# Tcadart/pyLatticeDSO

Hardware: AMD Instinct MI355X
Metric: beams/s assembly+PCG-solve (higher is better)
Workload: dtype f64

## Files before the change

pylatticedso_amd/csrc/pl_coarse.h:

```cpp
#pragma once
#include <hip/hip_runtime.h>

#include <algorithm>
#include <cstdint>
#include <cstdlib>
#include <vector>

#include "pl_dense.h"
#include "pl_kernels.h"
#include "pl_nodeword.h"
#include "pl_tile.h"

namespace pl {

constexpr int kDclMax = 256;
constexpr int kDclSlots = 4096;
inline bool node_words_enabled() {
  const char *e = std::getenv("PL_NODE_WORDS");
  return !(e && e[0] == '0');
}

struct Coarse {
  bool enabled = false;
  bool ready = false;
// ... 700 lines not shown
          mode_disp(q, rela, uA, tA);
          uA = mask3(uA, fa);
          tA = mask3(tA, fa >> 3);
        }
        if (inb) {
          mode_disp(q, relb, uB, tB);
          uB = mask3(uB, fb);
          tB = mask3(tB, fb >> 3);
        }
        V3 F, M;
        tip_force(r, uA, tA, uB, tB, F, M);
        double x6[6] = {0, 0, 0, 0, 0, 0};
        if (inb) {
          const V3 FB = mask3(F, fb), MB = mask3(M, fb >> 3);
          x6[0] += FB.x;
          x6[1] += FB.y;
          x6[2] += FB.z;
          x6[3] += MB.x + (relb[1] * FB.z - relb[2] * FB.y);
          x6[4] += MB.y + (relb[2] * FB.x - relb[0] * FB.z);
          x6[5] += MB.z + (relb[0] * FB.y - relb[1] * FB.x);
        }
        if (ina) {
          const V3 FA = mask3((-1.0) * F, fa), MA = mask3((-1.0) * M - cross(d, F), fa >> 3);
          x6[0] += FA.x;
          x6[1] += FA.y;
          x6[2] += FA.z;
          x6[3] += MA.x + (rela[1] * FA.z - rela[2] * FA.y);
          x6[4] += MA.y + (rela[2] * FA.x - rela[0] * FA.z);
          x6[5] += MA.z + (rela[0] * FA.y - rela[1] * FA.x);
        }
#pragma unroll
        for (int p = 0; p <= q; ++p) RR[q * (q + 1) / 2 + p] += x6[p];
      }
    }
  }
  const int lane = threadIdx.x & 63, wv = threadIdx.x >> 6;
  double *B = raw + (size_t)t * 144;
  if (RIGID) {
#pragma unroll
    for (int e = 0; e < 21; ++e) {
      const double s0 = wave_sum(RR[e]);
      if (lane == 0) red[e][wv] = s0;
    }
    __syncthreads();
    if (threadIdx.x < 21) {
      double v = 0.0;
#pragma unroll
      for (int q = 0; q < kBlock / kWave; ++q) v += red[threadIdx.x][q];
      int q = 0;
      while ((q + 1) * (q + 2) / 2 <= (int)threadIdx.x) ++q;
      const int p = (int)threadIdx.x - q * (q + 1) / 2;
      B[p * 12 + q] = v;
      B[q * 12 + p] = v;
    }
    return;
  }
#pragma unroll
  for (int e = 0; e < 21; ++e) {
    const double s1 = wave_sum(SS[e]);
    if (lane == 0) red[e][wv] = s1;
  }
#pragma unroll
  for (int e = 0; e < (RIGID ? 1 : 36); ++e) {
    const double s2 = wave_sum(RS[e]);
    if (lane == 0) red[21 + e][wv] = s2;
  }
  __syncthreads();
  if (threadIdx.x < 57) {
    double v = 0.0;
#pragma unroll
    for (int q = 0; q < kBlock / kWave; ++q) v += red[threadIdx.x][q];
    if (threadIdx.x < 21) {
      int q = 0;
      while ((q + 1) * (q + 2) / 2 <= (int)threadIdx.x) ++q;
      const int p = (int)threadIdx.x - q * (q + 1) / 2;
      B[(6 + p) * 12 + 6 + q] = v;
      B[(6 + q) * 12 + 6 + p] = v;
    } else {
      const int e = (int)threadIdx.x - 21, p = e / 6, q = e % 6;
      B[p * 12 + 6 + q] = v;
      B[(6 + q) * 12 + p] = v;
    }
  }
}
constexpr int kInv12Block = 192;
__global__ __launch_bounds__(kInv12Block) void k_tile_invert12(int64_t T, const double *__restrict__ raw,
                                                              double *__restrict__ Bt_inv) {
  constexpr int n = 12;
  __shared__ double A[n][n + 1];
  __shared__ double diag0[n];
  const int64_t t = blockIdx.x;
  if (t >= T) return;
  const int e = threadIdx.x, i = e / n, j = e - n * i;
  const bool act = e < n * n;
  if (act) A[i][j] = 0.5 * (raw[t * 144 + i * n + j] + raw[t * 144 + j * n + i]);
  __syncthreads();
  if (e < n) diag0[e] = A[e][e];
  __syncthreads();
  unsigned dropped = 0u;
  for (int k = 0; k < n; ++k) {
    const double d = A[k][k];
    if (!(d > 1e-10 * diag0[k]) || !(diag0[k] > 0.0)) {
      dropped |= 1u << k;
      continue;
    }
    const double inv = 1.0 / d;
    double v = 0.0;
    if (act) {
      const bool di = (dropped >> i) & 1u, dj = (dropped >> j) & 1u;
      if (i == k && j == k) v = -inv;
      else if (i == k) v = A[k][j] * inv;
      else if (j == k) v = A[k][i] * inv;
      else if (di || dj) v = A[i][j];
      else v = A[i][j] - (A[i][k] * inv) * A[k][j];
    }
    __syncthreads();
    if (act) A[i][j] = v;
    __syncthreads();
  }
  if (act) {
    const bool out = ((dropped >> i) & 1u) || ((dropped >> j) & 1u);
    Bt_inv[t * 144 + i * n + j] = out ? 0.0 : -A[i][j];
  }
}
inline void coarse_factor(Coarse &cs, int n, hipStream_t s, const std::function<void(int)> &after_chol, unsigned *bar,
                          TrtriPhases ph = TrtriPhases()) {
  if (cs.w16)
    dense_factor_inverse(cs.Ac, cs.Lf, reinterpret_cast<bf16_t *>(cs.W), reinterpret_cast<bf16_t *>(cs.Wt), cs.Dinv, n, n,
                         cs.info, cs.bw_blocks, s, after_chol, bar, ph);
  else
    dense_factor_inverse(cs.Ac, cs.Lf, cs.W, cs.Wt, cs.Dinv, n, n, cs.info, cs.bw_blocks, s, after_chol, bar, ph);
}
constexpr int kOneGemvMaxDofs = 2048;
inline void coarse_apply(const Coarse &cs, const double *r, double *t, double *y, double *dot_out, const double *add0,
                         hipStream_t s) {
  static const bool one_off = [] { const char *e = std::getenv("PL_ONE_GEMV"); return e && e[0] == '0'; }();
  if (cs.ainv_ready && cs.Ainv && cs.ncp <= kOneGemvMaxDofs && !one_off) {
    hipLaunchKernelGGL(k_full_gemv, dim3((cs.ncp + 3) / 4), dim3(kBlock), 0, s, cs.ncp, (const float *)cs.Ainv, cs.ncp, r, y,
                       dot_out, add0);
    return;
  }
  if (cs.w16)
    dense_apply(reinterpret_cast<const bf16_t *>(cs.W), reinterpret_cast<const bf16_t *>(cs.Wt), cs.ncp, cs.ncp, r, t, y,
                dot_out, add0, s);
  else
    dense_apply(cs.W, cs.Wt, cs.ncp, cs.ncp, r, t, y, dot_out, add0, s);
}

__global__ __launch_bounds__(kBlock) void k_to_float(int64_t n, const double *__restrict__ x, float *__restrict__ y) {
  const int64_t i = (int64_t)blockIdx.x * kBlock + threadIdx.x;
  if (i < n) y[i] = (float)x[i];
}

__device__ __forceinline__ void nword_rel(uint32_t w, double rscale, double &rx, double &ry, double &rz) {
  rx = (double)((int)(w << 24) >> 24) * rscale;
  ry = (double)((int)(w << 16) >> 24) * rscale;
  rz = (double)((int)(w << 8) >> 24) * rscale;
}

template <typename PT, typename RT, int TM = 6, bool MULTI = true, bool LOCAL = true>
__global__ __launch_bounds__(kBlock) void k_pcg_update_tile(const int32_t *__restrict__ tile_start,
                                                            const int32_t *__restrict__ agg_of_tile,
                                                            const double *__restrict__ cen,
                                                            const double *__restrict__ xyz,
                                                            const PT *__restrict__ Ap,
                                                            const float *__restrict__ dinv32,
                                                            const double *__restrict__ w ,
                                                            RT *__restrict__ r,
                                                            double *__restrict__ scal, double *__restrict__ rc,
                                                            const double *__restrict__ Bt_inv ,
                                                            double *__restrict__ yt,
                                                            const int32_t *__restrict__ aggL_of_tile ,
                                                            const double *__restrict__ cenL,
                                                            const uint8_t *__restrict__ shared ,
                                                            double *__restrict__ rcL, int ncp,
                                                            const uint8_t *__restrict__ skip_rows ,
                                                            int cm = 6 ,
                                                            const float *__restrict__ rel32 = nullptr ,
                                                            const uint32_t *__restrict__ nword = nullptr ,
                                                            const uint32_t *__restrict__ dtab = nullptr ,
                                                            double rscale = 0.0 ) {
  __shared__ double red[32][4 * kBlock / kWave];
  if constexpr (!MULTI) {
    w = nullptr;
    shared = nullptr;
  }
  if constexpr (!MULTI || !LOCAL) aggL_of_tile = nullptr;
  double *rr_slot = rc + ncp + (blockIdx.x & (kSlots - 1)), *rdr_slot = rr_slot + kSlots;
  const int t = blockIdx.x;
  double pap, old_rz;
  scalar_read2(scal, S_PAP, S_RZ_OLD, pap, old_rz);
  const double alpha = (pap != 0.0) ? old_rz / pap : 0.0;
  const int n0 = tile_start[t], n1 = tile_start[t + 1];
  const int a = agg_of_tile[t];
  const double c0 = cen[3 * a], c1 = cen[3 * a + 1], c2 = cen[3 * a + 2];
  __shared__ double sbi[16][TM];
  double bi[TM];
#pragma unroll
  for (int j = 0; j < TM; ++j) bi[j] = 0.0;
  const int my_mode = (TM == 12) ? ((int)threadIdx.x < 6 ? (int)threadIdx.x : ((int)threadIdx.x >= 8 && (int)threadIdx.x < 14
                                                                                   ? (int)threadIdx.x - 2 : -1))
                                 : ((int)threadIdx.x < 6 ? (int)threadIdx.x : -1);
  if (Bt_inv && my_mode >= 0) {
#pragma unroll
    for (int j = 0; j < TM; ++j) bi[j] = Bt_inv[(size_t)t * (TM * TM) + TM * my_mode + j];
  }
  if (threadIdx.x < 16) {
#pragma unroll
    for (int j = 0; j < TM; ++j) sbi[threadIdx.x][j] = bi[j];
  }
  double accS[6] = {0, 0, 0, 0, 0, 0};
  double accD[6] = {0, 0, 0, 0, 0, 0};
  double acc[8] = {0, 0, 0, 0, 0, 0, 0, 0};
  const int aL = aggL_of_tile ? aggL_of_tile[t] : 0;
  double l0 = 0.0, l1 = 0.0, l2 = 0.0;
  if (aggL_of_tile) {
    l0 = cenL[3 * aL];
    l1 = cenL[3 * aL + 1];
    l2 = cenL[3 * aL + 2];
  }
  double accL[6] = {0, 0, 0, 0, 0, 0};
  double accT[6] = {0, 0, 0, 0, 0, 0};
  const bool own_t = Bt_inv && shared;
  for (int i = n0 + threadIdx.x; i < n1; i += blockDim.x) {
    if (skip_rows && skip_rows[i]) continue;
    double av[6], dv[6], rv[6];
    const uint32_t nw = nword ? nword[i] : 0u;
    const float2 *d2 = dtab ? reinterpret_cast<const float2 *>(dtab + 8 * (nw >> 24))
                            : reinterpret_cast<const float2 *>(dinv32 + 6 * (int64_t)i);
#pragma unroll
    for (int k = 0; k < 3; ++k) {
      const double2 aa = load_pair(Ap, 3 * (int64_t)i + k), rr = load_pair(r, 3 * (int64_t)i + k);
      const float2 dd = d2[k];
      av[2 * k] = aa.x; av[2 * k + 1] = aa.y;
      dv[2 * k] = dd.x; dv[2 * k + 1] = dd.y;
      rv[2 * k] = rr.x; rv[2 * k + 1] = rr.y;
    }
#pragma unroll
    for (int k = 0; k < 6; ++k) rv[k] -= alpha * av[k];
#pragma unroll
    for (int k = 0; k < 3; ++k) store_pair(r, 3 * (int64_t)i + k, double2{rv[2 * k], rv[2 * k + 1]});
    if (sizeof(RT) == 4) {
#pragma unroll
      for (int k = 0; k < 6; ++k) rv[k] = (double)(float)rv[k];
    }
    double wt[6] = {1, 1, 1, 1, 1, 1};
    if (w) {
#pragma unroll
      for (int k = 0; k < 6; ++k) wt[k] = w[6 * (int64_t)i + k];
    }
    double rx, ry, rz;
    if (rscale != 0.0) {
      nword_rel(nw, rscale, rx, ry, rz);
    } else if (rel32) {
      rx = (double)rel32[3 * (int64_t)i];
      ry = (double)rel32[3 * (int64_t)i + 1];
      rz = (double)rel32[3 * (int64_t)i + 2];
    } else {
      rx = xyz[3 * (int64_t)i] - c0;
      ry = xyz[3 * (int64_t)i + 1] - c1;
      rz = xyz[3 * (int64_t)i + 2] - c2;
    }
    const double ru[3] = {wt[0] * rv[0], wt[1] * rv[1], wt[2] * rv[2]};
    acc[0] += ru[0];
    acc[1] += ru[1];
    acc[2] += ru[2];
    acc[3] += wt[3] * rv[3] + (ry * ru[2] - rz * ru[1]);
    acc[4] += wt[4] * rv[4] + (rz * ru[0] - rx * ru[2]);
    acc[5] += wt[5] * rv[5] + (rx * ru[1] - ry * ru[0]);
#pragma unroll
    for (int k = 0; k < 6; ++k) {
      acc[6] += wt[k] * rv[k] * rv[k];
      acc[7] += wt[k] * dv[k] * rv[k] * rv[k];
    }
    if (TM == 12 && cm == 12 && shared) {
      accD[0] += rx * ru[0];
      accD[1] += ry * ru[1];
      accD[2] += rz * ru[2];
      accD[3] += 0.5 * (ry * ru[0] + rx * ru[1]);
      accD[4] += 0.5 * (rz * ru[1] + ry * ru[2]);
      accD[5] += 0.5 * (rz * ru[0] + rx * ru[2]);
    }
    if (TM == 12 && !(shared && shared[i])) {
      accS[0] += rx * ru[0];
      accS[1] += ry * ru[1];
      accS[2] += rz * ru[2];
      accS[3] += 0.5 * (ry * ru[0] + rx * ru[1]);
      accS[4] += 0.5 * (rz * ru[1] + ry * ru[2]);
      accS[5] += 0.5 * (rz * ru[0] + rx * ru[2]);
    }
    if (own_t && !shared[i]) {
      accT[0] += rv[0];
      accT[1] += rv[1];
      accT[2] += rv[2];
      accT[3] += rv[3] + (ry * rv[2] - rz * rv[1]);
      accT[4] += rv[4] + (rz * rv[0] - rx * rv[2]);
      accT[5] += rv[5] + (rx * rv[1] - ry * rv[0]);
    }
    if (aggL_of_tile && !(shared && shared[i])) {
      const double sx = xyz[3 * (int64_t)i] - l0, sy = xyz[3 * (int64_t)i + 1] - l1, sz = xyz[3 * (int64_t)i + 2] - l2;
      accL[0] += rv[0];
      accL[1] += rv[1];
      accL[2] += rv[2];
      accL[3] += rv[3] + (sy * rv[2] - sz * rv[1]);
      accL[4] += rv[4] + (sz * rv[0] - sx * rv[2]);
      accL[5] += rv[5] + (sx * rv[1] - sy * rv[0]);
// ... 245 lines not shown
  unsigned long long h = 0x9E3779B97F4A7C15ull;
#pragma unroll
  for (int k = 0; k < 7; ++k) {
    h = (h ^ v[k]) * 0xBF58476D1CE4E5B9ull;
    h ^= h >> 29;
  }
  h *= 0x94D049BB133111EBull;
  h ^= h >> 32;
  return h == ~0ull ? 0 : h;
}
__device__ __forceinline__ int dcl_probe(unsigned long long h, unsigned long long *__restrict__ keys,
                                         int *__restrict__ owner, int i) {
  unsigned slot = (unsigned)(h >> 52) & (unsigned)(kDclSlots - 1);
  for (int probe = 0; probe < 32; ++probe) {
    unsigned long long cur = __hip_atomic_load(keys + slot, __ATOMIC_RELAXED, __HIP_MEMORY_SCOPE_AGENT);
    if (cur == ~0ull) cur = atomicCAS(keys + slot, ~0ull, h);
    if (cur == ~0ull || cur == h) {
      if (i < __hip_atomic_load(owner + slot, __ATOMIC_RELAXED, __HIP_MEMORY_SCOPE_AGENT)) atomicMin(owner + slot, i);
      return (int)slot;
    }
    slot = (slot + 1) & (unsigned)(kDclSlots - 1);
  }
  return -1;
}
__global__ __launch_bounds__(kBlock) void k_dcl_insert(int64_t N, const float *__restrict__ dinv,
                                                       const uint8_t *__restrict__ fixedbits,
                                                       unsigned long long *__restrict__ keys, int *__restrict__ owner,
                                                       uint16_t *__restrict__ slot_of_node, int *__restrict__ flags) {
  const int64_t i = (int64_t)blockIdx.x * kBlock + threadIdx.x;
  const bool valid = i < N;
  uint32_t v[7] = {0, 0, 0, 0, 0, 0, 0};
  if (valid) dcl_row(dinv, fixedbits, i, v);
  const unsigned long long h = valid ? dcl_hash(v) : 0ull;
  const int lane = threadIdx.x & 63;
  int found = -2;
  unsigned long long todo = __ballot(valid);
  for (int round = 0; round < 12 && todo; ++round) {
    const int leader = __ffsll((long long)todo) - 1;
    const unsigned long long hl =
        ((unsigned long long)(unsigned)__builtin_amdgcn_readlane((int)(h >> 32), leader) << 32) |
        (unsigned long long)(unsigned)__builtin_amdgcn_readlane((int)(h & 0xFFFFFFFFull), leader);
    const unsigned long long same = __ballot(valid && found == -2 && h == hl);
    int sl = 0;
    if (lane == leader) sl = dcl_probe(h, keys, owner, (int)i);
    sl = __builtin_amdgcn_readlane(sl, leader);
    if ((same >> lane) & 1ull) found = sl;
    todo &= ~same;
  }
  if (valid && found == -2) found = dcl_probe(h, keys, owner, (int)i);
  if (valid) {
    if (found < 0) flags[0] = 1;
    slot_of_node[i] = (uint16_t)(found < 0 ? 0 : found);
  }
}
__global__ __launch_bounds__(kBlock) void k_dcl_publish(int64_t N, const float *__restrict__ dinv,
                                                        const uint8_t *__restrict__ fixedbits,
                                                        const int *__restrict__ owner,
                                                        const uint16_t *__restrict__ slot_of_node,
                                                        int *__restrict__ dense_of_slot, uint32_t *__restrict__ table,
                                                        int *__restrict__ flags) {
  const int64_t i = (int64_t)blockIdx.x * kBlock + threadIdx.x;
  if (i >= N) return;
  const int slot = slot_of_node[i];
  if (owner[slot] != (int)i) return;
  const int d = atomicAdd(flags + 1, 1);
  if (d >= kDclMax) {
    flags[0] = 1;
    return;
  }
  uint32_t v[7];
  dcl_row(dinv, fixedbits, i, v);
#pragma unroll
  for (int k = 0; k < 7; ++k) table[8 * d + k] = v[k];
  table[8 * d + 7] = 0u;
  dense_of_slot[slot] = d;
}
__global__ __launch_bounds__(kBlock) void k_dcl_verify(int64_t N, const float *__restrict__ dinv,
                                                       const uint8_t *__restrict__ fixedbits,
                                                       const uint16_t *__restrict__ slot_of_node,
                                                       const int *__restrict__ dense_of_slot,
                                                       const uint32_t *__restrict__ table, uint32_t *__restrict__ nword,
                                                       int *__restrict__ flags) {
  const int64_t i = (int64_t)blockIdx.x * kBlock + threadIdx.x;
  if (i >= N) return;
  const int d = dense_of_slot[slot_of_node[i]];
  if (d < 0 || d >= kDclMax) {
    flags[0] = 1;
    return;
  }
  uint32_t v[7];
  dcl_row(dinv, fixedbits, i, v);
  bool same = true;
#pragma unroll
  for (int k = 0; k < 7; ++k) same = same && table[8 * d + k] == v[k];
  if (!same) {
    flags[0] = 1;
    return;
  }
  nword[i] = (nword[i] & 0x00FFFFFFu) | ((uint32_t)d << 24);
}
template <typename VT>
__global__ __launch_bounds__(kBlock) void k_condense_subtract(int64_t N, const uint8_t *__restrict__ cflag,
                                                              const VT *__restrict__ y, VT *__restrict__ r) {
  const int64_t t = (int64_t)blockIdx.x * kBlock + threadIdx.x;
  if (t >= 6 * N) return;
  if (!cflag[t / 6]) r[t] = (VT)((double)r[t] - (double)y[t]);
}
template <typename VT>
__global__ __launch_bounds__(kBlock) void k_condense_backsubst(int64_t nc, const int32_t *__restrict__ cnodes,
                                                               const double *__restrict__ inv,
                                                               const uint16_t *__restrict__ cls,
                                                               const VT *__restrict__ b,
                                                               const VT *__restrict__ y, VT *__restrict__ x) {
  const int64_t t = (int64_t)blockIdx.x * kBlock + threadIdx.x;
  const int64_t q = t / 6;
  const int k = (int)(t - 6 * q);
  if (q >= nc) return;
  const int64_t i = cnodes[q];
  const double *A = inv + 36 * (cls ? (int64_t)cls[q] : q);
  double acc = 0.0;
#pragma unroll
  for (int j = 0; j < 6; ++j) acc += A[6 * k + j] * ((double)b[6 * i + j] - (double)y[6 * i + j]);
  x[6 * i + k] = (VT)acc;
}

template <typename PT, typename RT, int TM = 6, bool MULTI = true, bool LOCAL = true>
__global__ __launch_bounds__(kBlock) void k_pcg_direction_coarse(const int32_t *__restrict__ tile_start,
                                                                 const RT *__restrict__ r,
                                                                 const float *__restrict__ dinv32,
                                                                 const double *__restrict__ xyz,
                                                                 const int32_t *__restrict__ agg_of_tile,
                                                                 const double *__restrict__ cen,
                                                                 const double *__restrict__ yc,
                                                                 const double *__restrict__ yt ,
                                                                 const uint8_t *__restrict__ fixedbits,
                                                                 PT *__restrict__ p, RT *__restrict__ x,
                                                                 const double *__restrict__ scal,
                                                                 double *__restrict__ scal_next,
                                                                 double *__restrict__ hist, int k,
                                                                 double *__restrict__ rc, int ncp,
                                                                 const int32_t *__restrict__ aggL_of_tile ,
                                                                 const double *__restrict__ cenL,
                                                                 const double *__restrict__ ycL,
                                                                 const uint8_t *__restrict__ shared ,
                                                                 double *__restrict__ rcL, int ncpL,
                                                                 const uint8_t *__restrict__ zero_rows ,
                                                                 int cm = 6,
                                                                 const float *__restrict__ rel32 = nullptr ,
                                                                 const uint32_t *__restrict__ nword = nullptr,
                                                                 const uint32_t *__restrict__ dtab = nullptr,
                                                                 double rscale = 0.0 ) {
  if constexpr (!MULTI) shared = nullptr;
  if constexpr (!MULTI || !LOCAL) aggL_of_tile = nullptr;
  double old, rz_new, pap;
  scalar_read3(scal, S_RZ_OLD, S_RZ_NEW, S_PAP, old, rz_new, pap);
  const double beta = (old != 0.0) ? rz_new / old : 0.0;
  const double alpha = (pap != 0.0) ? old / pap : 0.0;
  if (blockIdx.x == 1 || gridDim.x == 1)
    for (int e = threadIdx.x; e < ncp; e += blockDim.x) rc[e] = 0.0;
  if (aggL_of_tile && (blockIdx.x == 2 || gridDim.x <= 2))
    for (int e = threadIdx.x; e < ncpL; e += blockDim.x) rcL[e] = 0.0;
  if (blockIdx.x == 0 && threadIdx.x < kWave) {
    const int s = threadIdx.x;
    double rr = 0.0;
    for (int q = s; q < kSlots; q += kWave) rr += rc[ncp + q];
    rr = wave_sum(rr);
    if (s == 0) hist[k] = rr;
    for (int q = s; q < kSlots; q += kWave) {
      rc[ncp + q] = 0.0;
      rc[ncp + kSlots + q] = 0.0;
      scal_next[S_RZ_OLD * kSlots + q] = scal[S_RZ_NEW * kSlots + q];
      scal_next[S_RZ_NEW * kSlots + q] = 0.0;
      scal_next[S_PAP * kSlots + q] = 0.0;
    }
  }
  const int t = blockIdx.x;
  const int n0 = tile_start[t], n1 = tile_start[t + 1];
  const int a = agg_of_tile[t];
  const double *y = yc + cm * a;
  double U0 = y[0], U1 = y[1], U2 = y[2], W0 = y[3], W1 = y[4], W2 = y[5];
  double T[TM];
#pragma unroll
  for (int k = 0; k < TM; ++k) T[k] = 0.0;
  if (yt) {
    const double *q = yt + TM * (size_t)t;
#pragma unroll
    for (int k = 0; k < TM; ++k) T[k] = q[k];
    if (!shared) {
      U0 += T[0]; U1 += T[1]; U2 += T[2]; W0 += T[3]; W1 += T[4]; W2 += T[5];
    }
  }
  double ED[6] = {0, 0, 0, 0, 0, 0};
  if constexpr (TM == 12) {
    if (cm == 12) {
#pragma unroll
      for (int k = 0; k < 6; ++k) ED[k] = y[6 + k];
      if (!shared) {
#pragma unroll
        for (int k = 0; k < 6; ++k) {
          T[6 + k] += ED[k];
          ED[k] = 0.0;
        }
      }
    }
  }
  const bool own_t = yt && shared;
  const double c0 = cen[3 * a], c1 = cen[3 * a + 1], c2 = cen[3 * a + 2];
  double L[6] = {0, 0, 0, 0, 0, 0}, l0 = 0.0, l1 = 0.0, l2 = 0.0;
  if (aggL_of_tile) {
    const int aL = aggL_of_tile[t];
#pragma unroll
    for (int q = 0; q < 6; ++q) L[q] = ycL[6 * aL + q];
    l0 = cenL[3 * aL];
    l1 = cenL[3 * aL + 1];
    l2 = cenL[3 * aL + 2];
  }
  for (int64_t i = n0 + threadIdx.x; i < n1; i += blockDim.x) {
    if (zero_rows && zero_rows[i]) continue;
    const uint32_t nw = nword ? nword[i] : 0u;
    double rx, ry, rz;
    if (rscale != 0.0) {
      nword_rel(nw, rscale, rx, ry, rz);
    } else if (rel32) {
      rx = (double)rel32[3 * i];
      ry = (double)rel32[3 * i + 1];
      rz = (double)rel32[3 * i + 2];
    } else {
      rx = xyz[3 * i] - c0;
      ry = xyz[3 * i + 1] - c1;
      rz = xyz[3 * i + 2] - c2;
    }
    double zc[6] = {U0 + (W1 * rz - W2 * ry), U1 + (W2 * rx - W0 * rz), U2 + (W0 * ry - W1 * rx), W0, W1, W2};
    if constexpr (TM == 12) {
     if (shared && cm == 12) {
      zc[0] += ED[0] * rx + 0.5 * (ED[3] * ry + ED[5] * rz);
      zc[1] += ED[1] * ry + 0.5 * (ED[3] * rx + ED[4] * rz);
      zc[2] += ED[2] * rz + 0.5 * (ED[4] * ry + ED[5] * rx);
     }
     if (!(shared && shared[i])) {
      zc[0] += T[6] * rx + 0.5 * (T[9] * ry + T[11] * rz);
      zc[1] += T[7] * ry + 0.5 * (T[9] * rx + T[10] * rz);
      zc[2] += T[8] * rz + 0.5 * (T[10] * ry + T[11] * rx);
     }
    }
    if (own_t && !shared[i]) {
      zc[0] += T[0] + (T[4] * rz - T[5] * ry);
      zc[1] += T[1] + (T[5] * rx - T[3] * rz);
      zc[2] += T[2] + (T[3] * ry - T[4] * rx);
      zc[3] += T[3];
      zc[4] += T[4];
      zc[5] += T[5];
    }
    if (aggL_of_tile && !(shared && shared[i])) {
      const double sx = xyz[3 * i] - l0, sy = xyz[3 * i + 1] - l1, sz = xyz[3 * i + 2] - l2;
      zc[0] += L[0] + (L[4] * sz - L[5] * sy);
      zc[1] += L[1] + (L[5] * sx - L[3] * sz);
      zc[2] += L[2] + (L[3] * sy - L[4] * sx);
      zc[3] += L[3];
      zc[4] += L[4];
      zc[5] += L[5];
    }
    const uint32_t *row = dtab ? dtab + 8 * (nw >> 24) : nullptr;
    const unsigned fb = dtab ? row[6] : (unsigned)fixedbits[i];
    const float2 *d2 = dtab ? reinterpret_cast<const float2 *>(row) : reinterpret_cast<const float2 *>(dinv32 + 6 * i);
#pragma unroll
    for (int q = 0; q < 3; ++q) {
      const double2 rr = load_pair(r, 3 * i + q);
      const float2 dd = d2[q];
      double2 pp = load_pair(p, 3 * i + q);
      double2 xx = load_pair(x, 3 * i + q);
      xx.x += alpha * pp.x;
      xx.y += alpha * pp.y;
      store_pair(x, 3 * i + q, xx);
      const double z0 = dd.x * rr.x + (((fb >> (2 * q)) & 1u) ? 0.0 : zc[2 * q]);
      const double z1 = dd.y * rr.y + (((fb >> (2 * q + 1)) & 1u) ? 0.0 : zc[2 * q + 1]);
      pp.x = z0 + beta * pp.x;
      pp.y = z1 + beta * pp.y;
      store_pair(p, 3 * i + q, pp);
    }
  }
}

template <typename PT, typename RT, int TM>
__global__ __launch_bounds__(kBlock) void k_pcg_direction_flat(int64_t N, const int32_t *__restrict__ tile_of_node,
                                                               const RT *__restrict__ r,
                                                               const float *__restrict__ dinv32,
                                                               const double *__restrict__ xyz,
                                                               const int32_t *__restrict__ agg_of_tile,
                                                               const double *__restrict__ cen,
                                                               const double *__restrict__ yc,
                                                               const double *__restrict__ yt ,
                                                               const uint8_t *__restrict__ fixedbits,
                                                               PT *__restrict__ p, RT *__restrict__ x,
                                                               const double *__restrict__ scal,
                                                               double *__restrict__ scal_next,
                                                               double *__restrict__ hist, int k,
                                                               double *__restrict__ rc, int ncp,
                                                               const int32_t *__restrict__ keep ,
                                                               int cm, const uint8_t *__restrict__ shared ,
                                                               const float *__restrict__ rel32 = nullptr ,
                                                               const uint32_t *__restrict__ nword = nullptr,
                                                               const uint32_t *__restrict__ dtab = nullptr,
                                                               double rscale = 0.0 ) {
  double old, rz_new, pap;
  scalar_read3(scal, S_RZ_OLD, S_RZ_NEW, S_PAP, old, rz_new, pap);
  const double beta = (old != 0.0) ? rz_new / old : 0.0;
  const double alpha = (pap != 0.0) ? old / pap : 0.0;
  if (blockIdx.x == 1 || gridDim.x == 1)
    for (int e = threadIdx.x; e < ncp; e += blockDim.x) rc[e] = 0.0;
  if (blockIdx.x == 0 && threadIdx.x < kWave) {
    const int s = threadIdx.x;
    double rr = 0.0;
    for (int q = s; q < kSlots; q += kWave) rr += rc[ncp + q];
    rr = wave_sum(rr);
    if (s == 0) hist[k] = rr;
    for (int q = s; q < kSlots; q += kWave) {
      rc[ncp + q] = 0.0;
      rc[ncp + kSlots + q] = 0.0;
      scal_next[S_RZ_OLD * kSlots + q] = scal[S_RZ_NEW * kSlots + q];
      scal_next[S_RZ_NEW * kSlots + q] = 0.0;
      scal_next[S_PAP * kSlots + q] = 0.0;
    }
  }
  const int64_t lane_pair = (int64_t)blockIdx.x * blockDim.x + threadIdx.x;
  if (lane_pair >= 3 * N) return;
  const int64_t slot = lane_pair / 3;
  const int q = (int)(lane_pair - 3 * slot);
  const int64_t i = keep ? (int64_t)keep[slot] : slot;
  const int64_t pair = 3 * i + q;
  const int t = tile_of_node[i];
  const int a = agg_of_tile[t];
  const double *y = yc + cm * a;
  double C[12];
#pragma unroll
  for (int m = 0; m < 6; ++m) C[m] = y[m];
#pragma unroll
  for (int m = 6; m < 12; ++m) C[m] = 0.0;
  if constexpr (TM == 12) {
    if (cm == 12) {
#pragma unroll
      for (int m = 6; m < 12; ++m) C[m] = y[m];
    }
  }
  if (yt && !(shared && shared[i])) {
    const double *w = yt + TM * (size_t)t;
#pragma unroll
    for (int m = 0; m < TM; ++m) C[m] += w[m];
  }
  const uint32_t nw = nword ? nword[i] : 0u;
  double rx, ry, rz;
  if (rscale != 0.0) {
    nword_rel(nw, rscale, rx, ry, rz);
  } else if (rel32) {
    rx = (double)rel32[3 * i];
    ry = (double)rel32[3 * i + 1];
    rz = (double)rel32[3 * i + 2];
  } else {
    rx = xyz[3 * i] - cen[3 * a];
    ry = xyz[3 * i + 1] - cen[3 * a + 1];
    rz = xyz[3 * i + 2] - cen[3 * a + 2];
  }
  double zc[6] = {C[0] + (C[4] * rz - C[5] * ry), C[1] + (C[5] * rx - C[3] * rz), C[2] + (C[3] * ry - C[4] * rx),
                  C[3], C[4], C[5]};
  if constexpr (TM == 12) {
    zc[0] += C[6] * rx + 0.5 * (C[9] * ry + C[11] * rz);
    zc[1] += C[7] * ry + 0.5 * (C[9] * rx + C[10] * rz);
    zc[2] += C[8] * rz + 0.5 * (C[10] * ry + C[11] * rx);
  }
  double z0 = q == 0 ? zc[0] : (q == 1 ? zc[2] : zc[4]);
  double z1 = q == 0 ? zc[1] : (q == 1 ? zc[3] : zc[5]);
  const uint32_t *row = dtab ? dtab + 8 * (nw >> 24) : nullptr;
  const unsigned fb = dtab ? row[6] : (unsigned)fixedbits[i];
  const float2 dd = dtab ? reinterpret_cast<const float2 *>(row)[q] : reinterpret_cast<const float2 *>(dinv32)[pair];
  const double2 rr = load_pair(r, pair);
  double2 pp = load_pair(p, pair);
  double2 xx = load_pair(x, pair);
  xx.x += alpha * pp.x;
  xx.y += alpha * pp.y;
  store_pair(x, pair, xx);
  z0 = dd.x * rr.x + (((fb >> (2 * q)) & 1u) ? 0.0 : z0);
  z1 = dd.y * rr.y + (((fb >> (2 * q + 1)) & 1u) ? 0.0 : z1);
  pp.x = z0 + beta * pp.x;
  pp.y = z1 + beta * pp.y;
  store_pair(p, pair, pp);
}

}
```

pylatticedso_amd/csrc/pl_solver.h:

```cpp
#pragma once
#include <type_traits>

#include "pl_assembly.h"
#include "pl_schedule.h"
#include "pl_warm.h"

namespace {

int read_slots(pl_context *c, const double *dev, double *sum) {
  double h[pl::kSlots];
  PL_HIP(hipMemcpyAsync(h, dev, sizeof(h), hipMemcpyDeviceToHost, c->stream));
  PL_HIP(hipStreamSynchronize(c->stream));
  *sum = 0.0;
  for (int k = 0; k < pl::kSlots; ++k) *sum += h[k];
  return PL_OK;
}

int solve_begin(pl_context *c, const double *bb_slots, pl_stats_t *st, double *bb, bool *zero) {
  *zero = false;
  const int rc = read_slots(c, bb_slots, bb);
  if (rc) return rc;
  st->b_norm = std::sqrt(*bb);
  st->iterations = 0;
  st->converged = 0;
  st->rel_residual = 0.0;
  if (*bb > 0.0) return PL_OK;
  *zero = true;
  st->converged = 1;
  return std::isnan(*bb) ? fail(PL_ERR_NAN, "NaN in the right-hand side") : PL_OK;
}

inline void converged_at(pl_stats_t *st, int iterations, double stop_reason) {
  st->converged = 1;
  st->iterations = iterations;
  st->info = 0.0;
  st->stop_reason = stop_reason;
}

template <int V>
using Int = std::integral_constant<int, V>;

template <typename F>
inline void with_tile_modes(const pl_context *c, F &&f) {
  if (tile_modes_now(c) == 12) f(Int<12>{});
  else f(Int<6>{});
}
template <typename F>
inline void with_tail_variant(const pl_context *c, F &&f) {
  with_tile_modes(c, [&](auto tm) {
    if (c->coarseL.ready) f(tm, std::true_type{}, std::true_type{});
    else if (c->dist.active) f(tm, std::true_type{}, std::false_type{});
    else f(tm, std::false_type{}, std::false_type{});
  });
}

struct NodeWords {
  const float *rel32;
  const uint32_t *nword, *dtab;
  double rscale;
};
inline NodeWords node_words_of(const pl_context *c) {
  const pl::Coarse &cs = c->coarse;
  const bool words = node_words_apply(c);
  NodeWords nw;
  nw.rel32 = cs.rel_exact ? (const float *)cs.rel32.p : (const float *)nullptr;
  nw.dtab = words && cs.dcl_ready ? (const uint32_t *)cs.dcl_table : (const uint32_t *)nullptr;
  nw.rscale = words && cs.rel_e >= 0 ? std::ldexp(1.0, -cs.rel_e) : 0.0;
  nw.nword = (nw.dtab || nw.rscale != 0.0) ? (const uint32_t *)cs.nword.p : (const uint32_t *)nullptr;
  return nw;
}

template <typename PT, typename RT, int TM, bool MULTI, bool LOCAL>
void launch_update_tile(pl_context *c, Int<TM>, std::bool_constant<MULTI>, std::bool_constant<LOCAL>, const PT *Ap, RT *r,
                        double *scal, double *rc_out, const NodeWords &nw) {
  pl::Coarse &cs = c->coarse, &cl = c->coarseL;
  hipLaunchKernelGGL((pl::k_pcg_update_tile<PT, RT, TM, MULTI, LOCAL>), dim3((unsigned)cs.n_tiles), dim3(cs.vblock), 0,
                     c->stream, c->tile.tile_start.p, cs.agg_of_tile.p, cs.cen.p, c->xyz.p, Ap, cs.dinv32,
                     c->dist.active ? (const double *)c->dist.weight.p : (const double *)nullptr, r, scal, rc_out,
                     cs.tile_level ? (const double *)cs.Bt_inv : (const double *)nullptr, cs.yt,
                     LOCAL ? (const int32_t *)cl.agg_of_tile.p : (const int32_t *)nullptr,
                     LOCAL ? (const double *)cl.cen.p : (const double *)nullptr,
                     MULTI ? (const uint8_t *)c->sharedbits.p : (const uint8_t *)nullptr, LOCAL ? cl.rc : (double *)nullptr,
                     cs.ncp, c->cond_use ? (const uint8_t *)c->cflag.p : (const uint8_t *)nullptr, cs.cm, nw.rel32, nw.nword,
                     nw.dtab, nw.rscale);
}
template <typename PT, typename RT, int TM, bool MULTI, bool LOCAL>
void launch_direction_coarse(pl_context *c, Int<TM>, std::bool_constant<MULTI>, std::bool_constant<LOCAL>, PT *p, RT *x,
                             const RT *r, double *cur, double *nxt, int hist_slot, const NodeWords &nw) {
  pl::Coarse &cs = c->coarse, &cl = c->coarseL;
  hipLaunchKernelGGL((pl::k_pcg_direction_coarse<PT, RT, TM, MULTI, LOCAL>), dim3((unsigned)cs.n_tiles), dim3(cs.vblock), 0,
                     c->stream, c->tile.tile_start.p, r, cs.dinv32, c->xyz.p, cs.agg_of_tile.p, cs.cen.p, cs.yc,
                     cs.tile_level ? (const double *)cs.yt : (const double *)nullptr, c->fixedbits.p, p, x, cur, nxt,
                     c->hist.p, hist_slot, cs.rc, cs.ncp,
                     LOCAL ? (const int32_t *)cl.agg_of_tile.p : (const int32_t *)nullptr,
                     LOCAL ? (const double *)cl.cen.p : (const double *)nullptr,
                     LOCAL ? (const double *)cl.yc : (const double *)nullptr,
                     MULTI ? (const uint8_t *)c->sharedbits.p : (const uint8_t *)nullptr, LOCAL ? cl.rc : (double *)nullptr,
                     LOCAL ? cl.ncp : 0, c->cond_use ? (const uint8_t *)c->cflag.p : (const uint8_t *)nullptr, cs.cm,
                     nw.rel32, nw.nword, nw.dtab, nw.rscale);
}
template <typename PT, typename RT, int TM>
void launch_direction_flat(pl_context *c, Int<TM>, PT *p, RT *x, const RT *r, double *cur, double *nxt, int hist_slot,
                           const NodeWords &nw) {
  pl::Coarse &cs = c->coarse;
  const int64_t n_flat = c->cond_use ? c->N - c->n_cond : c->N;
  hipLaunchKernelGGL((pl::k_pcg_direction_flat<PT, RT, TM>), dim3((unsigned)((3 * n_flat + pl::kBlock - 1) / pl::kBlock)),
                     dim3(pl::kBlock), 0, c->stream, n_flat, cs.tile_of_node.p, r, cs.dinv32, c->xyz.p, cs.agg_of_tile.p,
                     cs.cen.p, cs.yc, cs.tile_level ? (const double *)cs.yt : (const double *)nullptr, c->fixedbits.p, p, x,
                     cur, nxt, c->hist.p, hist_slot, cs.rc, cs.ncp,
                     c->cond_use ? (const int32_t *)c->ckeep.p : (const int32_t *)nullptr, cs.cm,
                     c->dist.active ? (const uint8_t *)c->sharedbits.p : (const uint8_t *)nullptr, nw.rel32, nw.nword, nw.dtab,
                     nw.rscale);
}

template <typename PT, typename RT>
int pcg_tail_coarse_t(pl_context *c, double *cur, double *nxt, int hist_slot, PT *p, const PT *Ap, RT *x, RT *r) {
  pl::Coarse &cs = c->coarse, &cl = c->coarseL;
  const bool useL = cl.ready;
  const NodeWords nw = node_words_of(c);
  with_tail_variant(c, [&](auto tm, auto multi, auto local) { launch_update_tile(c, tm, multi, local, Ap, r, cur, cs.rc, nw); });
  if (useL)
    pl::coarse_apply(cl, cl.rc, cl.tv, cl.yc, cs.rc + cs.ncp + pl::kSlots, (const double *)nullptr, c->stream);
  if (c->dist.active) {
    if (pl::dist_sum_scalars(c->dist, cs.rc, cs.ncp + 2 * pl::kSlots, c->stream))
      return fail(PL_ERR_HIP, "RCCL all-reduce of the coarse residual failed");
  }
  pl::coarse_apply(cs, cs.rc, cs.tv, cs.yc, cur + pl::S_RZ_NEW * pl::kSlots, cs.rc + cs.ncp + pl::kSlots, c->stream);
  if (!useL && sizeof(PT) == 8)
    with_tile_modes(c, [&](auto tm) { launch_direction_flat(c, tm, p, x, (const RT *)r, cur, nxt, hist_slot, nw); });
  else
    with_tail_variant(c, [&](auto tm, auto multi, auto local) {
      launch_direction_coarse(c, tm, multi, local, p, x, (const RT *)r, cur, nxt, hist_slot, nw);
    });
  PL_HIP(hipGetLastError());
  return PL_OK;
}

int pcg_tail_coarse(pl_context *c, double *cur, double *nxt, int hist_slot) {
  return pcg_tail_coarse_t<double, double>(c, cur, nxt, hist_slot, c->p.p, (const double *)c->Ap.p, c->x.p, c->r.p);
}

inline void ddm_precondition(pl_context *c, double *dot, bool restricted = false) {
  if (c->dd2_ready) {
    pl::Coarse &cs = c->dd2;
    const uint8_t *fx = c->have_bc ? (const uint8_t *)c->fixed.p : (const uint8_t *)nullptr;
    if (!restricted)
      hipLaunchKernelGGL(pl::k_ddm_restrict, dim3((unsigned)c->dd2_n_agg), dim3(pl::kBlock), 0, c->stream, c->dd2_ptr.p,
                         c->dd2_nodes.p, (const double *)c->dd2_cen.p, (const double *)c->dd2_xyz.p, fx,
                         (const double *)c->r.p, cs.rc);
    pl::coarse_apply(cs, cs.rc, cs.tv, cs.yc, dot, (const double *)nullptr, c->stream);
    hipLaunchKernelGGL(pl::k_ddm_two_level_apply, dim3(grid_for(c->N * 6)), dim3(pl::kBlock), 0, c->stream, c->N,
                       (const double *)c->dd_B.p, c->dd2_agg.p, (const double *)c->dd2_cen.p, (const double *)c->dd2_xyz.p, fx,
                       (const double *)cs.yc, (const double *)c->r.p, c->z.p, dot, cs.rc, cs.ncp);
    return;
  }
  if (c->dd_ready)
    pl::dense_apply(c->dd_W.p, c->dd_Wt.p, c->dd_n, c->dd_n, c->r.p, c->dd_tv.p, c->z.p, dot, (const double *)nullptr,
                    c->stream);
  else
    hipLaunchKernelGGL(pl::k_ddm_node_blocks_apply, dim3(grid_for(c->N * 6)), dim3(pl::kBlock), 0, c->stream, c->N,
                       (const double *)c->dd_B.p, (const double *)c->r.p, c->z.p, dot);
}

inline int small_set_size() { return pl::S_COUNT * pl::kSlots; }
inline double *small_set(pl_context *c, int k) { return c->small_scal.p + (size_t)((k + 4) & 3) * small_set_size(); }
inline double *small_rc(pl_context *c, int parity) { return c->small_rc.p + (size_t)(parity & 1) * (c->coarse.ncp + 2 * pl::kSlots); }

int small_prepare(pl_context *c) {
  const int64_t n6 = c->N * 6;
  const size_t nrc = 2 * (size_t)(c->coarse.ncp + 2 * pl::kSlots);
  if (!c->p2.p || c->p2.n < (size_t)n6) PL_HIP(c->p2.alloc((size_t)n6));
  if (!c->small_scal.p) PL_HIP(c->small_scal.alloc(4 * (size_t)small_set_size()));
  if (!c->small_rc.p || c->small_rc.n < nrc) PL_HIP(c->small_rc.alloc(nrc));
  PL_HIP(hipMemsetAsync(c->small_scal.p, 0, 4 * (size_t)small_set_size() * sizeof(double), c->stream));
  PL_HIP(hipMemsetAsync(c->small_rc.p, 0, nrc * sizeof(double), c->stream));
  PL_HIP(hipMemsetAsync(c->p.p, 0, n6 * sizeof(double), c->stream));
  PL_HIP(hipMemsetAsync(c->p2.p, 0, n6 * sizeof(double), c->stream));
  return PL_OK;
}

template <int TM>
void launch_small_z(pl_context *c, Int<TM>, int k, int hist_slot) {
  pl::Coarse &cs = c->coarse;
  hipLaunchKernelGGL((pl::k_small_z<TM>), dim3((unsigned)cs.n_tiles), dim3(cs.vblock), 0, c->stream, c->tile.tile_start.p,
                     cs.agg_of_tile.p, cs.cen.p, c->xyz.p, (const double *)c->r.p, cs.dinv32, c->fixedbits.p,
                     c->cond_use ? (const uint8_t *)c->cflag.p : (const uint8_t *)nullptr, (const float *)cs.Ainv, cs.ncp, cs.cm,
                     (const double *)small_rc(c, k + 1), small_rc(c, k),
                     cs.tile_level ? (const double *)cs.yt : (const double *)nullptr, c->z.p, small_set(c, k + 1),
                     small_set(c, k + 2), c->hist.p, hist_slot);
}
int small_tail(pl_context *c, int k, int hist_slot) {
  const NodeWords none = {(const float *)nullptr, (const uint32_t *)nullptr, (const uint32_t *)nullptr, 0.0};
  with_tile_modes(c, [&](auto tm) {
    launch_update_tile(c, tm, std::false_type{}, std::false_type{}, (const double *)c->Ap.p, c->r.p, small_set(c, k),
                       small_rc(c, k + 1), none);
    launch_small_z(c, tm, k, hist_slot);
  });
  PL_HIP(hipGetLastError());
  return PL_OK;
}

inline double *small_p_of(pl_context *c, int k) { return (k & 1) ? c->p2.p : c->p.p; }

int small_iteration(pl_context *c, int k) {
  pl::Defer df;
  df.z = c->z.p;
  df.p_old = small_p_of(c, k - 1);
  df.p_new = small_p_of(c, k);
  df.xsol = c->x.p;
  df.sc_prev = small_set(c, k - 1);
  df.sc_cur = small_set(c, k);
  double *dot = small_set(c, k) + pl::S_PAP * pl::kSlots;
  const bool stream_form = !c->pal_lds;
  const uint32_t *vw = stream_form ? c->vword_dir.p : c->vword.p;
  const void *tab = stream_form ? (const void *)c->tile.dir_table.p : (const void *)c->pal_dense.p;
  const int n_tab = stream_form ? c->tile.n_dir : c->pal_entries;
  const pl::Rec5 *r5 = stream_form ? reinterpret_cast<const pl::Rec5 *>(c->rec5.p) : (const pl::Rec5 *)nullptr;
  if (c->cond_use) {
    const pl::CondSolve cs = cond_solve(c, pl::kEndsCondensedSolve);
    if (!pl::launch_tile_spmv_lds_defer(c->tile, vw, tab, n_tab, r5, nullptr, df.p_new, nullptr, c->stream,
                                        pl::kEndsCondensedSolve, c->cflag.p, cs, df))
      return fail(PL_ERR_STATE, "short iteration: the LDS-resident K*p does not fit this lattice");
    int rc = launch_spmv(c, df.p_new, c->Ap.p, true, dot, c->maskC.p, pl::kEndsOthers);
    if (rc) return rc;
  } else {
    if (!pl::launch_tile_spmv_lds_defer(c->tile, vw, tab, n_tab, r5, c->fixedbits.p, c->Ap.p, dot, c->stream, pl::kEndsAll,
                                        nullptr, pl::CondSolve(), df))
      return fail(PL_ERR_STATE, "short iteration: the LDS-resident K*p does not fit this lattice");
  }
  return small_tail(c, k, k);
}

int small_finish(pl_context *c, int K) {
  if (K <= 0) return PL_OK;
  hipLaunchKernelGGL(pl::k_small_final_x, dim3(grid_stream(c->N * 6)), dim3(pl::kBlock), 0, c->stream, c->N,
                     c->cond_use ? (const uint8_t *)c->cflag.p : (const uint8_t *)nullptr,
                     (const double *)small_p_of(c, K - 1), (const double *)small_set(c, K - 1), c->x.p);
  PL_HIP(hipGetLastError());
  return PL_OK;
}

inline void periodic_average(pl_context *c, double *v) {
  if (c->n_per_groups > 0)
    hipLaunchKernelGGL(pl::k_periodic_average, dim3(grid_for(6 * c->n_per_groups)), dim3(pl::kBlock), 0, c->stream,
                       c->n_per_groups, c->per_ptr.p, c->per_nodes.p, v);
}

int pcg_iteration(pl_context *c, int k) {
  if (c->small_use) return small_iteration(c, k);
  const int64_t n6 = c->N * 6;
  const int set = pl::S_COUNT * pl::kSlots;
  double *cur = c->scal.p + (k & 1) * set, *nxt = c->scal.p + ((k + 1) & 1) * set;
  int rc = apply_operator(c, c->p.p, c->Ap.p, cur + pl::S_PAP * pl::kSlots);
  if (rc) return rc;
  if (c->coarse.ready) return pcg_tail_coarse(c, cur, nxt, k);
  periodic_average(c, c->Ap.p);
  const bool ref = ref_cg(c) && !c->dist.active;
  const bool restart = ref && c->opt.restart_every > 0 && k > 0 && (k % c->opt.restart_every) == 0;
  const bool has_M = c->dd_ready || c->dd_blocks || c->opt.precond >= 1;
  const double *pn = c->p.p, *psrc = nullptr;
  if (restart) {
    if (has_M) {
      PL_HIP(hipMemcpyAsync(c->tmp.p, c->z.p, n6 * sizeof(double), hipMemcpyDeviceToDevice, c->stream));
      pn = psrc = c->tmp.p;
    } else {
// ... 598 lines not shown
```

Measured before the change: 257.4 million.

## Prefetch node operands before scalar reductions and add wave-uniform tile coefficient path

Both PCG direction kernels now issue their per-node loads (r, p, x, diagonal inverse, fixed bits, node words) before the wave reduction of the CG scalars, so memory latency overlaps the reductions. The scalar read is changed to a per-lane slot load plus wave_sum. The flat kernel also reads agg_of_node directly and, when every lane in a wave belongs to the same tile, uses readfirstlane-based uniform loads of the coarse and tile coefficients, which can be switched off through PL_UNIFORM_TILE. The cost is higher register pressure from holding the prefetched values, plus an extra load of the uniform coefficients that goes unused when the wave is not uniform.

```diff
diff --git a/pylatticedso_amd/csrc/pl_coarse.h b/pylatticedso_amd/csrc/pl_coarse.h
--- a/pylatticedso_amd/csrc/pl_coarse.h
+++ b/pylatticedso_amd/csrc/pl_coarse.h
@@ -876,6 +876,16 @@
   if (i < n) y[i] = (float)x[i];
 }
 
+__device__ __forceinline__ double2 load_raw(const double *v, int64_t pair) { return reinterpret_cast<const double2 *>(v)[pair]; }
+__device__ __forceinline__ float2 load_raw(const float *v, int64_t pair) { return reinterpret_cast<const float2 *>(v)[pair]; }
+__device__ __forceinline__ double2 widen(double2 a) { return a; }
+__device__ __forceinline__ double2 widen(float2 a) {
+  asm volatile("" : "+v"(a.x), "+v"(a.y));
+  return {(double)a.x, (double)a.y};
+}
+template <typename T>
+using raw_pair_t = decltype(load_raw((const T *)nullptr, 0));
+
 __device__ __forceinline__ void nword_rel(uint32_t w, double rscale, double &rx, double &ry, double &rz) {
   rx = (double)((int)(w << 24) >> 24) * rscale;
   ry = (double)((int)(w << 16) >> 24) * rscale;
@@ -1427,8 +1437,39 @@
                                                                  double rscale = 0.0 ) {
   if constexpr (!MULTI) shared = nullptr;
   if constexpr (!MULTI || !LOCAL) aggL_of_tile = nullptr;
-  double old, rz_new, pap;
-  scalar_read3(scal, S_RZ_OLD, S_RZ_NEW, S_PAP, old, rz_new, pap);
+  static_assert(kSlots == kWave, "one slot per lane");
+  const int t = blockIdx.x;
+  const int n0 = tile_start[t], n1 = tile_start[t + 1];
+  unsigned skip = 0u, sh = 0u, fb = 0u;
+  uint32_t word = 0u;
+  raw_pair_t<RT> rr[3], xx[3];
+  raw_pair_t<PT> pp[3];
+  float2 dn[3] = {{0.f, 0.f}, {0.f, 0.f}, {0.f, 0.f}};
+  const auto request = [&](int64_t i) {
+    if (zero_rows) {
+      skip = zero_rows[i];
+      if (skip) return;
+    }
+    if (nword) word = nword[i];
+    if (shared) sh = shared[i];
+#pragma unroll
+    for (int q = 0; q < 3; ++q) {
+      rr[q] = load_raw(r, 3 * i + q);
+      pp[q] = load_raw(p, 3 * i + q);
+      xx[q] = load_raw(x, 3 * i + q);
+    }
+    const uint32_t *row = dtab ? dtab + 8 * (word >> 24) : nullptr;
+    fb = dtab ? row[6] : (unsigned)fixedbits[i];
+    const float2 *d2 = dtab ? reinterpret_cast<const float2 *>(row) : reinterpret_cast<const float2 *>(dinv32 + 6 * i);
+#pragma unroll
+    for (int q = 0; q < 3; ++q) dn[q] = d2[q];
+  };
+  int64_t i = n0 + threadIdx.x;
+  bool requested = i < n1;
+  if (requested) request(i);
+  const int sl = threadIdx.x & 63;
+  const double s_old = scal[S_RZ_OLD * kSlots + sl], s_new = scal[S_RZ_NEW * kSlots + sl], s_pap = scal[S_PAP * kSlots + sl];
+  const double old = wave_sum(s_old), rz_new = wave_sum(s_new), pap = wave_sum(s_pap);
   const double beta = (old != 0.0) ? rz_new / old : 0.0;
   const double alpha = (pap != 0.0) ? old / pap : 0.0;
   if (blockIdx.x == 1 || gridDim.x == 1)
@@ -1449,8 +1490,6 @@
       scal_next[S_PAP * kSlots + q] = 0.0;
     }
   }
-  const int t = blockIdx.x;
-  const int n0 = tile_start[t], n1 = tile_start[t + 1];
   const int a = agg_of_tile[t];
   const double *y = yc + cm * a;
   double U0 = y[0], U1 = y[1], U2 = y[2], W0 = y[3], W1 = y[4], W2 = y[5];
@@ -1480,7 +1519,6 @@
     }
   }
   const bool own_t = yt && shared;
-  const double c0 = cen[3 * a], c1 = cen[3 * a + 1], c2 = cen[3 * a + 2];
   double L[6] = {0, 0, 0, 0, 0, 0}, l0 = 0.0, l1 = 0.0, l2 = 0.0;
   if (aggL_of_tile) {
     const int aL = aggL_of_tile[t];
@@ -1490,20 +1528,21 @@
     l1 = cenL[3 * aL + 1];
     l2 = cenL[3 * aL + 2];
   }
-  for (int64_t i = n0 + threadIdx.x; i < n1; i += blockDim.x) {
-    if (zero_rows && zero_rows[i]) continue;
-    const uint32_t nw = nword ? nword[i] : 0u;
+  for (; i < n1; i += blockDim.x) {
+    if (!requested) request(i);
+    requested = false;
+    if (skip) continue;
     double rx, ry, rz;
     if (rscale != 0.0) {
-      nword_rel(nw, rscale, rx, ry, rz);
+      nword_rel(word, rscale, rx, ry, rz);
     } else if (rel32) {
       rx = (double)rel32[3 * i];
       ry = (double)rel32[3 * i + 1];
       rz = (double)rel32[3 * i + 2];
     } else {
-      rx = xyz[3 * i] - c0;
-      ry = xyz[3 * i + 1] - c1;
-      rz = xyz[3 * i + 2] - c2;
+      rx = xyz[3 * i] - cen[3 * a];
+      ry = xyz[3 * i + 1] - cen[3 * a + 1];
+      rz = xyz[3 * i + 2] - cen[3 * a + 2];
     }
     double zc[6] = {U0 + (W1 * rz - W2 * ry), U1 + (W2 * rx - W0 * rz), U2 + (W0 * ry - W1 * rx), W0, W1, W2};
     if constexpr (TM == 12) {
@@ -1512,13 +1551,13 @@
       zc[1] += ED[1] * ry + 0.5 * (ED[3] * rx + ED[4] * rz);
       zc[2] += ED[2] * rz + 0.5 * (ED[4] * ry + ED[5] * rx);
      }
-     if (!(shared && shared[i])) {
+     if (sh == 0u) {
       zc[0] += T[6] * rx + 0.5 * (T[9] * ry + T[11] * rz);
       zc[1] += T[7] * ry + 0.5 * (T[9] * rx + T[10] * rz);
       zc[2] += T[8] * rz + 0.5 * (T[10] * ry + T[11] * rx);
      }
     }
-    if (own_t && !shared[i]) {
+    if (own_t && sh == 0u) {
       zc[0] += T[0] + (T[4] * rz - T[5] * ry);
       zc[1] += T[1] + (T[5] * rx - T[3] * rz);
       zc[2] += T[2] + (T[3] * ry - T[4] * rx);
@@ -1526,7 +1565,7 @@
       zc[4] += T[4];
       zc[5] += T[5];
     }
-    if (aggL_of_tile && !(shared && shared[i])) {
+    if (aggL_of_tile && sh == 0u) {
       const double sx = xyz[3 * i] - l0, sy = xyz[3 * i + 1] - l1, sz = xyz[3 * i + 2] - l2;
       zc[0] += L[0] + (L[4] * sz - L[5] * sy);
       zc[1] += L[1] + (L[5] * sx - L[3] * sz);
@@ -1535,23 +1574,19 @@
       zc[4] += L[4];
       zc[5] += L[5];
     }
-    const uint32_t *row = dtab ? dtab + 8 * (nw >> 24) : nullptr;
-    const unsigned fb = dtab ? row[6] : (unsigned)fixedbits[i];
-    const float2 *d2 = dtab ? reinterpret_cast<const float2 *>(row) : reinterpret_cast<const float2 *>(dinv32 + 6 * i);
 #pragma unroll
     for (int q = 0; q < 3; ++q) {
-      const double2 rr = load_pair(r, 3 * i + q);
-      const float2 dd = d2[q];
-      double2 pp = load_pair(p, 3 * i + q);
-      double2 xx = load_pair(x, 3 * i + q);
-      xx.x += alpha * pp.x;
-      xx.y += alpha * pp.y;
-      store_pair(x, 3 * i + q, xx);
-      const double z0 = dd.x * rr.x + (((fb >> (2 * q)) & 1u) ? 0.0 : zc[2 * q]);
-      const double z1 = dd.y * rr.y + (((fb >> (2 * q + 1)) & 1u) ? 0.0 : zc[2 * q + 1]);
-      pp.x = z0 + beta * pp.x;
-      pp.y = z1 + beta * pp.y;
-      store_pair(p, 3 * i + q, pp);
+      const double2 dd = widen(dn[q]);
+      const double2 rq = widen(rr[q]);
+      double2 pq = widen(pp[q]), xq = widen(xx[q]);
+      xq.x += alpha * pq.x;
+      xq.y += alpha * pq.y;
+      store_pair(x, 3 * i + q, xq);
+      const double z0 = dd.x * rq.x + (((fb >> (2 * q)) & 1u) ? 0.0 : zc[2 * q]);
+      const double z1 = dd.y * rq.y + (((fb >> (2 * q + 1)) & 1u) ? 0.0 : zc[2 * q + 1]);
+      pq.x = z0 + beta * pq.x;
+      pq.y = z1 + beta * pq.y;
+      store_pair(p, 3 * i + q, pq);
     }
   }
 }
@@ -1561,7 +1596,7 @@
                                                                const RT *__restrict__ r,
                                                                const float *__restrict__ dinv32,
                                                                const double *__restrict__ xyz,
-                                                               const int32_t *__restrict__ agg_of_tile,
+                                                               const int32_t *__restrict__ agg_of_node,
                                                                const double *__restrict__ cen,
                                                                const double *__restrict__ yc,
                                                                const double *__restrict__ yt ,
@@ -1573,56 +1608,57 @@
                                                                double *__restrict__ rc, int ncp,
                                                                const int32_t *__restrict__ keep ,
                                                                int cm, const uint8_t *__restrict__ shared ,
+                                                               int uniform_ok,
                                                                const float *__restrict__ rel32 = nullptr ,
                                                                const uint32_t *__restrict__ nword = nullptr,
                                                                const uint32_t *__restrict__ dtab = nullptr,
                                                                double rscale = 0.0 ) {
-  double old, rz_new, pap;
-  scalar_read3(scal, S_RZ_OLD, S_RZ_NEW, S_PAP, old, rz_new, pap);
+  static_assert(kSlots == kWave, "one slot per lane");
+  const int64_t lane_pair = (int64_t)blockIdx.x * blockDim.x + threadIdx.x;
+  const bool live = lane_pair < 3 * N;
+  const int64_t lp = live ? lane_pair : 3 * N - 1;
+  const int64_t slot = lp / 3;
+  const int q = (int)(lp - 3 * slot);
+  const int64_t i = keep ? (int64_t)keep[slot] : slot;
+  const int64_t pair = 3 * i + q;
+  const int sl = threadIdx.x & 63;
+  const double s_old = scal[S_RZ_OLD * kSlots + sl], s_new = scal[S_RZ_NEW * kSlots + sl], s_pap = scal[S_PAP * kSlots + sl];
+  const uint32_t nw = nword ? nword[i] : 0u;
+  const int t = tile_of_node[i];
+  const int a = agg_of_node[i];
+  const unsigned sh = shared ? (unsigned)shared[i] : 0u;
+  const raw_pair_t<RT> rr_raw = load_raw(r, pair), xx_raw = load_raw(x, pair);
+  const raw_pair_t<PT> pp_raw = load_raw(p, pair);
+  float2 dd = {0.f, 0.f};
+  unsigned fb = 0u;
+  if (!dtab) {
+    dd = reinterpret_cast<const float2 *>(dinv32)[pair];
+    fb = (unsigned)fixedbits[i];
+  }
+  const double old = wave_sum(s_old), rz_new = wave_sum(s_new), pap = wave_sum(s_pap);
   const double beta = (old != 0.0) ? rz_new / old : 0.0;
   const double alpha = (pap != 0.0) ? old / pap : 0.0;
   if (blockIdx.x == 1 || gridDim.x == 1)
     for (int e = threadIdx.x; e < ncp; e += blockDim.x) rc[e] = 0.0;
   if (blockIdx.x == 0 && threadIdx.x < kWave) {
     const int s = threadIdx.x;
-    double rr = 0.0;
-    for (int q = s; q < kSlots; q += kWave) rr += rc[ncp + q];
-    rr = wave_sum(rr);
-    if (s == 0) hist[k] = rr;
-    for (int q = s; q < kSlots; q += kWave) {
-      rc[ncp + q] = 0.0;
-      rc[ncp + kSlots + q] = 0.0;
-      scal_next[S_RZ_OLD * kSlots + q] = scal[S_RZ_NEW * kSlots + q];
-      scal_next[S_RZ_NEW * kSlots + q] = 0.0;
-      scal_next[S_PAP * kSlots + q] = 0.0;
-    }
-  }
-  const int64_t lane_pair = (int64_t)blockIdx.x * blockDim.x + threadIdx.x;
-  if (lane_pair >= 3 * N) return;
-  const int64_t slot = lane_pair / 3;
-  const int q = (int)(lane_pair - 3 * slot);
-  const int64_t i = keep ? (int64_t)keep[slot] : slot;
-  const int64_t pair = 3 * i + q;
-  const int t = tile_of_node[i];
-  const int a = agg_of_tile[t];
-  const double *y = yc + cm * a;
-  double C[12];
-#pragma unroll
-  for (int m = 0; m < 6; ++m) C[m] = y[m];
-#pragma unroll
-  for (int m = 6; m < 12; ++m) C[m] = 0.0;
-  if constexpr (TM == 12) {
-    if (cm == 12) {
-#pragma unroll
-      for (int m = 6; m < 12; ++m) C[m] = y[m];
-    }
-  }
-  if (yt && !(shared && shared[i])) {
-    const double *w = yt + TM * (size_t)t;
-#pragma unroll
-    for (int m = 0; m < TM; ++m) C[m] += w[m];
-  }
-  const uint32_t nw = nword ? nword[i] : 0u;
+    double rr0 = 0.0;
+    for (int e = s; e < kSlots; e += kWave) rr0 += rc[ncp + e];
+    rr0 = wave_sum(rr0);
+    if (s == 0) hist[k] = rr0;
+    for (int e = s; e < kSlots; e += kWave) {
+      rc[ncp + e] = 0.0;
+      rc[ncp + kSlots + e] = 0.0;
+      scal_next[S_RZ_OLD * kSlots + e] = scal[S_RZ_NEW * kSlots + e];
+      scal_next[S_RZ_NEW * kSlots + e] = 0.0;
+      scal_next[S_PAP * kSlots + e] = 0.0;
+    }
+  }
+  if (dtab) {
+    const uint32_t *row = dtab + 8 * (nw >> 24);
+    fb = row[6];
+    dd = reinterpret_cast<const float2 *>(row)[q];
+  }
   double rx, ry, rz;
   if (rscale != 0.0) {
     nword_rel(nw, rscale, rx, ry, rz);
@@ -1635,6 +1671,67 @@
     ry = xyz[3 * i + 1] - cen[3 * a + 1];
     rz = xyz[3 * i + 2] - cen[3 * a + 2];
   }
+  const int t0 = __builtin_amdgcn_readfirstlane(t), a0 = __builtin_amdgcn_readfirstlane(a);
+  const bool uniform = uniform_ok && !shared && __all(t == t0);
+  double Yu[12], Wu[12];
+  {
+    const double *__restrict__ y = yc + cm * a0;
+#pragma unroll
+    for (int m = 0; m < 6; ++m) Yu[m] = y[m];
+#pragma unroll
+    for (int m = 6; m < 12; ++m) Yu[m] = 0.0;
+    if constexpr (TM == 12) {
+      if (cm == 12) {
+#pragma unroll
+        for (int m = 6; m < 12; ++m) Yu[m] = y[m];
+      }
+    }
+#pragma unroll
+    for (int m = 0; m < 12; ++m) Wu[m] = 0.0;
+    if (yt) {
+      const double *__restrict__ w = yt + TM * (size_t)t0;
+#pragma unroll
+      for (int m = 0; m < TM; ++m) Wu[m] = w[m];
+    }
+  }
+  if (!live) return;
+  const double2 rr = widen(rr_raw);
+  double2 pp = widen(pp_raw), xx = widen(xx_raw);
+  xx.x += alpha * pp.x;
+  xx.y += alpha * pp.y;
+  store_pair(x, pair, xx);
+  double C[12];
+  if (uniform) {
+#pragma unroll
+    for (int m = 0; m < 12; ++m) C[m] = Yu[m];
+    if (yt) {
+#pragma unroll
+      for (int m = 0; m < TM; ++m) C[m] += Wu[m];
+    }
+  } else {
+    const double *__restrict__ y = yc + cm * a;
+#pragma unroll
+    for (int m = 0; m < 6; ++m) C[m] = y[m];
+#pragma unroll
+    for (int m = 6; m < 12; ++m) C[m] = 0.0;
+    if constexpr (TM == 12) {
+      if (cm == 12) {
+#pragma unroll
+        for (int m = 6; m < 12; ++m) C[m] = y[m];
+      }
+    }
+    if (yt && sh == 0u) {
+      const double *__restrict__ w = yt + TM * (size_t)t;
+#pragma unroll
+      for (int m = 0; m < TM; ++m) {
+        if (m > 0 && m % 4 == 0) {
+          asm volatile("" ::: "memory");
+          __builtin_amdgcn_sched_barrier(0);
+        }
+        C[m] += w[m];
+      }
+    }
+  }
   double zc[6] = {C[0] + (C[4] * rz - C[5] * ry), C[1] + (C[5] * rx - C[3] * rz), C[2] + (C[3] * ry - C[4] * rx),
                   C[3], C[4], C[5]};
   if constexpr (TM == 12) {
@@ -1644,15 +1741,6 @@
   }
   double z0 = q == 0 ? zc[0] : (q == 1 ? zc[2] : zc[4]);
   double z1 = q == 0 ? zc[1] : (q == 1 ? zc[3] : zc[5]);
-  const uint32_t *row = dtab ? dtab + 8 * (nw >> 24) : nullptr;
-  const unsigned fb = dtab ? row[6] : (unsigned)fixedbits[i];
-  const float2 dd = dtab ? reinterpret_cast<const float2 *>(row)[q] : reinterpret_cast<const float2 *>(dinv32)[pair];
-  const double2 rr = load_pair(r, pair);
-  double2 pp = load_pair(p, pair);
-  double2 xx = load_pair(x, pair);
-  xx.x += alpha * pp.x;
-  xx.y += alpha * pp.y;
-  store_pair(x, pair, xx);
   z0 = dd.x * rr.x + (((fb >> (2 * q)) & 1u) ? 0.0 : z0);
   z1 = dd.y * rr.y + (((fb >> (2 * q + 1)) & 1u) ? 0.0 : z1);
   pp.x = z0 + beta * pp.x;
diff --git a/pylatticedso_amd/csrc/pl_solver.h b/pylatticedso_amd/csrc/pl_solver.h
--- a/pylatticedso_amd/csrc/pl_solver.h
+++ b/pylatticedso_amd/csrc/pl_solver.h
@@ -99,18 +99,22 @@
                      LOCAL ? cl.ncp : 0, c->cond_use ? (const uint8_t *)c->cflag.p : (const uint8_t *)nullptr, cs.cm,
                      nw.rel32, nw.nword, nw.dtab, nw.rscale);
 }
+inline bool uniform_tile_waves() {
+  const char *e = std::getenv("PL_UNIFORM_TILE");
+  return !(e && e[0] == '0');
+}
 template <typename PT, typename RT, int TM>
 void launch_direction_flat(pl_context *c, Int<TM>, PT *p, RT *x, const RT *r, double *cur, double *nxt, int hist_slot,
                            const NodeWords &nw) {
   pl::Coarse &cs = c->coarse;
   const int64_t n_flat = c->cond_use ? c->N - c->n_cond : c->N;
   hipLaunchKernelGGL((pl::k_pcg_direction_flat<PT, RT, TM>), dim3((unsigned)((3 * n_flat + pl::kBlock - 1) / pl::kBlock)),
-                     dim3(pl::kBlock), 0, c->stream, n_flat, cs.tile_of_node.p, r, cs.dinv32, c->xyz.p, cs.agg_of_tile.p,
+                     dim3(pl::kBlock), 0, c->stream, n_flat, cs.tile_of_node.p, r, cs.dinv32, c->xyz.p, cs.agg_of_node.p,
                      cs.cen.p, cs.yc, cs.tile_level ? (const double *)cs.yt : (const double *)nullptr, c->fixedbits.p, p, x,
                      cur, nxt, c->hist.p, hist_slot, cs.rc, cs.ncp,
                      c->cond_use ? (const int32_t *)c->ckeep.p : (const int32_t *)nullptr, cs.cm,
-                     c->dist.active ? (const uint8_t *)c->sharedbits.p : (const uint8_t *)nullptr, nw.rel32, nw.nword, nw.dtab,
-                     nw.rscale);
+                     c->dist.active ? (const uint8_t *)c->sharedbits.p : (const uint8_t *)nullptr, uniform_tile_waves() ? 1 : 0,
+                     nw.rel32, nw.nword, nw.dtab, nw.rscale);
 }
 
 template <typename PT, typename RT>
```

After: 261.7 million (median of 6 runs). 1.02x the previous value.
